# Thomasedv/RRIN

Hardware: AMD Instinct MI355X
Metric: interpolated frames/sec at 1280x720 fp32 (Net.forward, frame pairs/s) (higher is better)
Workload: dtype f32

## Files before the change

rrin_amd/csrc/conv_winoc42.hip:

```cpp
#include <type_traits>

#include "common.hpp"

#ifndef RRIN_WINO42_AGPR
#define RRIN_WINO42_AGPR 0
#endif
namespace rrin {

typedef float w42f16 __attribute__((ext_vector_type(16)));
typedef float w42f4 __attribute__((ext_vector_type(4)));

template <int PCW_>
struct W42 {
  static constexpr int PCW = PCW_;
  static constexpr int PRW = 32 / PCW;
  static constexpr int TW = 4 * PCW;
  static constexpr int TH = 2 * PRW;
  static constexpr int RC = TW + 2;
  static constexpr int WM = (RC + 3) / 4;
  static constexpr int RW = PCW == 8 ? 36 : 22;
  static_assert(RW >= 4 * WM, "raw row slots");
  static constexpr int RG = (TH + 2) * RW;
  static constexpr int RAW = 2 * RG;
  static constexpr int PIECES = (RAW + 255) / 256;
  static constexpr int STAGE = PIECES * 256;
  static constexpr int NS = 3;
  static constexpr int XP = 65;
  static constexpr int XREC = 4 * 16 * XP;
  static constexpr size_t LDS = (size_t)(NS * STAGE > XREC ? NS * STAGE : XREC) * 16;
};
static_assert(W42<8>::LDS == kWinoC42Lds && W42<4>::LDS == kWinoC42Lds, "LDS size (common.hpp)");
static_assert(2 * kWinoC42Lds <= 160 * 1024, "two blocks per CU");
struct W42P {
  static constexpr int XP = 66;
  static constexpr int XREC = 4 * 8 * XP;
  static constexpr size_t LDS = (size_t)(XREC + W42<8>::NS * W42<8>::STAGE) * 16;
};
static_assert(2 * W42P::LDS <= 160 * 1024, "two blocks per CU (persistent)");

template <int WM>
__device__ constexpr int w42_slot(int col) { return (col & 3) * WM + (col >> 2); }

__device__ inline __amdgpu_buffer_rsrc_t w42_rsrc(const void* base) {
  const uint64_t p = (uint64_t)base;
  const uint64_t u = ((uint64_t)(uint32_t)__builtin_amdgcn_readfirstlane((int)(p >> 32)) << 32) |
                     (uint32_t)__builtin_amdgcn_readfirstlane((int)(uint32_t)p);
  return __builtin_amdgcn_make_buffer_rsrc((void*)u, 0, 0x7fffffff, 0x00020000);
}

template <int EPI, int PCW, bool PERSIST>
__global__ __launch_bounds__(256, 2) void conv3x3_winoc42_kernel(ConvH8Args a) {
  using G = W42<PCW>;
  static_assert(!PERSIST || PCW == 8, "persistent tiles: the 32 x 8 geometry");
  constexpr int TH = G::TH, TW = G::TW, RG = G::RG, RW = G::RW, STAGE = G::STAGE, P = G::PIECES, WM = G::WM;
  constexpr int SB = PERSIST ? W42P::XREC : 0;
  extern __shared__ __attribute__((aligned(16))) uint4 smem4[];
  const int tid = threadIdx.x, lane = tid & 63;
  const int yw = __builtin_amdgcn_readfirstlane(tid >> 6);
  const int j = lane & 31, hh = lane >> 5;
  const int pc = j % PCW, pr = j / PCW;
  int bid;
  {
    const int nwg = (int)gridDim.x, q = nwg >> 3, r = nwg & 7;
    const int xcd = blockIdx.x & 7, slot = blockIdx.x >> 3;
    bid = (xcd < r ? xcd * (q + 1) : r * (q + 1) + (xcd - r) * q) + slot;
  }
  const int ntiles = a.co_blocks * a.tiles_x * a.tiles_y * a.n;
  if (bid >= ntiles) return;
  const int nch = a.nchunks;
  auto decode = [&](int tile, int& cob_, int& x0_, int& y0_, int& img_) {
    const int cpg = a.cob_group > 0 ? a.cob_group : a.co_blocks;
    const int gsz = cpg * (ntiles / a.co_blocks);
    const int g = tile / gsz;
    const int r = tile - g * gsz;
    const int cg = min(cpg, a.co_blocks - g * cpg);
    cob_ = g * cpg + r % cg;
    int t = r / cg;
    x0_ = (t % a.tiles_x) * TW;
    t /= a.tiles_x;
    y0_ = (t % a.tiles_y) * TH;
    img_ = t / a.tiles_y;
  };
  int tile = bid, cob, x0, y0, img;
  decode(tile, cob, x0, y0, img);

  auto tile_base = [&](int img_, int y0_, int x0_) {
    return a.src_hi + (int64_t)img_ * a.src_img + (int64_t)y0_ * a.src_wp + x0_ + (kH8PadLeft - 1);
  };
  const uint4* tbase = tile_base(img, y0, x0);
  static_assert(P <= 4, "DMA pieces");
  uint32_t voff[4];
#pragma unroll
  for (int it = 0; it < P; ++it) {
    const int idx = tid + 256 * it;
    const int g = idx >= RG ? 1 : 0;
    const int rem = idx < G::RAW ? idx - g * RG : 0;
    const int r = rem / RW, pos = rem - r * RW;
    const int m = pos / WM, q = pos - m * WM;
    const int col = 4 * q + m;
    const bool ok = idx < G::RAW && m < 4 && col < G::RC;
    voff[it] = ok ? (uint32_t)((int64_t)g * a.src_gp + (int64_t)r * a.src_wp + col) * 16u : 0u;
  }
  const int64_t chunk_stride = 2 * a.src_gp;
  auto issue_raw_at = [&](const uint4* base, int s) {
    const auto rs = w42_rsrc(base);
#pragma unroll
    for (int it = 0; it < P; ++it)
      __builtin_amdgcn_raw_ptr_buffer_load_lds(
          rs, (__attribute__((address_space(3))) void*)(smem4 + SB + s * STAGE + 256 * it + 64 * yw), 16, voff[it], 0, 0,
          0);
  };
  const uint4* raw_next = tbase;

  auto u_base = [&](int cob_) { return a.w_hi + (int64_t)cob_ * nch * 1536; };
  const uint4* ub = u_base(cob);
  const uint32_t uvoff = (uint32_t)(hh * 32 + j) * 16u;
  auto load_u = [&](int c, int x) {
    const int soff = c * (1536 * 16) + (6 * yw + (x & 4)) * 1024;
    return __builtin_bit_cast(w42f4,
                              __builtin_amdgcn_raw_buffer_load_b128(w42_rsrc(ub), uvoff + (x & 3) * 1024, soff, 0));
  };

  const int ra = yw == 0 ? 0 : (yw == 2 ? 2 : 1);
  const int rb = yw == 0 ? 2 : (yw == 1 ? 2 : (yw == 2 ? 1 : 3));
  const float sg = yw == 1 ? 1.f : -1.f;
  const int lbase = hh * RG + 2 * pr * RW + pc;
  const int oa = lbase + ra * RW, ob = lbase + rb * RW;

  w42f16 acc[6];
  w42f4 ua[6];
  w42f4 v[6];
  w42f4 d[12];

  auto read_raw = [&](int s) {
    const uint4* rw = smem4 + SB + s * STAGE;
#pragma unroll
    for (int k = 0; k < 6; ++k) {
      d[2 * k] = __builtin_bit_cast(w42f4, rw[oa + w42_slot<WM>(k)]);
      d[2 * k + 1] = __builtin_bit_cast(w42f4, rw[ob + w42_slot<WM>(k)]);
    }
  };
  w42f4 t[6];
  auto rows = [&]() {
#pragma unroll
    for (int k = 0; k < 6; ++k)
#pragma unroll
      for (int e = 0; e < 4; ++e) t[k][e] = fmaf(sg, d[2 * k + 1][e], d[2 * k][e]);
  };
  auto cols_a = [&]() {
#pragma unroll
    for (int e = 0; e < 4; ++e) {
      v[0][e] = fmaf(4.f, t[0][e], fmaf(-5.f, t[2][e], t[4][e]));
      v[1][e] = fmaf(-4.f, t[1][e] + t[2][e], t[3][e] + t[4][e]);
      v[2][e] = fmaf(4.f, t[1][e] - t[2][e], t[4][e] - t[3][e]);
    }
  };
  auto cols_b = [&]() {
#pragma unroll
    for (int e = 0; e < 4; ++e) {
      const float p = t[1][e] - t[3][e], s = t[4][e] - t[2][e];
      v[3][e] = fmaf(-2.f, p, s);
      v[4][e] = fmaf(2.f, p, s);
      v[5][e] = fmaf(4.f, t[1][e], fmaf(-5.f, t[3][e], t[5][e]));
    }
  };
  auto mfma_point = [&](const w42f4(&u)[6], int x, const bool first) {
#pragma unroll
    for (int e = 0; e < 4; ++e)
      acc[x] = __builtin_amdgcn_mfma_f32_32x32x2f32(u[x][e], v[x][e], first && e == 0 ? w42f16{} : acc[x], 0, 0, 0);
  };
  auto bar = [&]() { asm volatile("s_waitcnt lgkmcnt(0)\n\ts_barrier" ::: "memory"); };
  auto fence = [&]() { __builtin_amdgcn_sched_barrier(0); };

  auto chunk = [&](int c, int s, const bool more, const bool first, w42f4(&u)[6]) {
    const int cu = c + 1;
#pragma unroll
    for (int x = 0; x < 3; ++x) {
      mfma_point(u, x, first);
      if (more) u[x] = load_u(cu, x);
      fence();
    }
    if (more) {
      if (first)
        RRIN_VMWAIT(0, 9);
      else
        RRIN_VMWAIT(0, 6);
      bar();
      issue_raw_at(raw_next, s == 0 ? 2 : s - 1);
      if (c + 3 < nch) raw_next += chunk_stride;
      read_raw(s == 2 ? 0 : s + 1);
    }
    fence();
    mfma_point(u, 3, first);
    if (more) u[3] = load_u(cu, 3);
    fence();
    mfma_point(u, 4, first);
    if (more) u[4] = load_u(cu, 4);
    fence();
    if (more) {
      rows();
      cols_a();
    }
    fence();
    mfma_point(u, 5, first);
    if (more) u[5] = load_u(cu, 5);
    fence();
    if (more) cols_b();
  };
  auto next_stage = [](int s) { return s == 2 ? 0 : s + 1; };

  auto issue_prologue_raw = [&]() {
    issue_raw_at(tbase, 0);
    issue_raw_at(nch > 1 ? tbase + chunk_stride : tbase, 1);
    vm_fence();
  };
  auto issue_prologue_u = [&]() {
#pragma unroll
    for (int x = 0; x < 6; ++x) ua[x] = load_u(0, x);
    vm_fence();
  };
  issue_prologue_raw();
  issue_prologue_u();

  constexpr int NPR = 32 / TW;
  const int xo = lane & (TW - 1), cx = xo & 3;
  const int prw = yw * NPR + (NPR == 1 ? 0 : (lane >> 4) & 1);
  const int src = (xo >> 2) + PCW * prw + 32 * hh;
  auto qrec = [&](int k) {
    w42f4 g;
#pragma unroll
    for (int e = 0; e < 4; ++e) {
      const int vi = 4 * k + e, c = vi >> 4, i = vi & 15;
      const float m0 = acc[0][i], m1 = acc[1][i], m2 = acc[2][i], m3 = acc[3][i], m4 = acc[4][i], m5 = acc[5][i];
      g[e] = c == 0   ? (m0 + (m1 + m2)) + (m3 + m4)
             : c == 1 ? fmaf(2.f, m3 - m4, m1 - m2)
             : c == 2 ? fmaf(4.f, m3 + m4, m1 + m2)
                      : fmaf(8.f, m3 - m4, m1 - m2) + m5;
    }
    return g;
  };
  w42f4* X = reinterpret_cast<w42f4*>(smem4);
  float bsv[16];
  int ncob = 0;
  auto epilogue = [&](auto pf) {
    float yv[2][16];
    if constexpr (!PERSIST) {
      constexpr int XP = G::XP;
#pragma unroll
      for (int k = 0; k < 16; ++k) X[(yw * 16 + k) * XP + lane] = qrec(k);
      __syncthreads();
#pragma unroll
      for (int k4 = 0; k4 < 4; ++k4) {
        const int k = 4 * cx + k4;
        const w42f4 q0 = X[(0 * 16 + k) * XP + src];
        const w42f4 q1 = X[(1 * 16 + k) * XP + src];
        const w42f4 q2 = X[(2 * 16 + k) * XP + src];
        const w42f4 q3 = X[(3 * 16 + k) * XP + src];
#pragma unroll
        for (int e = 0; e < 4; ++e) {
          yv[0][4 * k4 + e] = (q0[e] + q1[e]) + q2[e];
          yv[1][4 * k4 + e] = (q1[e] - q2[e]) - q3[e];
        }
      }
    } else {
      constexpr int XP = W42P::XP;
#pragma unroll
      for (int h = 0; h < 2; ++h) {
#pragma unroll
        for (int kk = 0; kk < 8; ++kk) X[(yw * 8 + kk) * XP + lane] = qrec(4 * (kk >> 1) + 2 * h + (kk & 1));
        __syncthreads();
#pragma unroll
        for (int k4h = 0; k4h < 2; ++k4h) {
          const int kk = 2 * cx + k4h, k4 = 2 * h + k4h;
          const w42f4 q0 = X[(0 * 8 + kk) * XP + src];
          const w42f4 q1 = X[(1 * 8 + kk) * XP + src];
          const w42f4 q2 = X[(2 * 8 + kk) * XP + src];
          const w42f4 q3 = X[(3 * 8 + kk) * XP + src];
#pragma unroll
          for (int e = 0; e < 4; ++e) {
            yv[0][4 * k4 + e] = (q0[e] + q1[e]) + q2[e];
            yv[1][4 * k4 + e] = (q1[e] - q2[e]) - q3[e];
          }
        }
        if (h == 0) __syncthreads();
      }
      if constexpr (decltype(pf)::value) {
        ub = u_base(ncob);
        issue_prologue_u();
      }
    }
    uint4* dst = a.dst_hi + (int64_t)img * a.dst_img;
    auto store4 = [&](int64_t rec, const float* vv) {
      dst[rec] = make_uint4(__float_as_uint(vv[0]), __float_as_uint(vv[1]), __float_as_uint(vv[2]), __float_as_uint(vv[3]));
    };
    const int x = x0 + xo, yb = y0 + 2 * prw;
    if constexpr (EPI == RRIN_EPI_SUBPIXEL) {
      const int HH = 2 * a.h, WW = 2 * a.w, creal = a.cout >> 2;
  #pragma unroll
      for (int r = 0; r < 2; ++r) {
        const int y = yb + r;
        if (cob * 32 < a.cout && y < a.h && x < a.w) {
  #pragma unroll
          for (int qq = 0; qq < 4; ++qq) {
            const int Y = 2 * y + (qq >> 1), XX = 2 * x + (qq & 1);
            const int64_t ri = ring_index(Y, XX, HH, WW);
            if (ri >= 0) {
  #pragma unroll
              for (int e = 0; e < 4; ++e)
                a.edge[((int64_t)img * creal + cob * 8 + 4 * hh + e) * a.ring + ri] = yv[r][4 * qq + e];
            } else {
              float vv[4];
  #pragma unroll
              for (int e = 0; e < 4; ++e) vv[e] = yv[r][4 * qq + e] + bsv[4 * qq + e];
              store4((int64_t)(2 * cob + hh) * a.dst_gp + (int64_t)(Y + 1) * a.dst_wp + XX + kH8PadLeft, vv);
            }
          }
        }
      }
    } else {
      float vv[2][16];
  #pragma unroll
      for (int r = 0; r < 2; ++r) {
        const int y = yb + r;
  #pragma unroll
        for (int i = 0; i < 16; ++i) {
          float tv = yv[r][i] + bsv[i];
          if constexpr (EPI != RRIN_EPI_LINEAR) tv = leaky(tv, a.slope);
          vv[r][i] = tv;
        }
  #pragma unroll
        for (int qq = 0; qq < 4; ++qq) {
          if (cob * 32 + 8 * qq < a.cout && y < a.h && x < a.w) {
            const int64_t rec = (int64_t)(cob * 8 + 2 * qq + hh) * a.dst_gp + (int64_t)(y + 1) * a.dst_wp + x + kH8PadLeft;
            store4(rec, &vv[r][4 * qq]);
            if constexpr (EPI == RRIN_EPI_LEAKY_REP) {
              const int dy0 = y == 0 ? -1 : 0, dy1 = y == a.h - 1 ? 1 : 0;
              const int dx0 = x == 0 ? -1 : 0, dx1 = x == a.w - 1 ? 1 : 0;
              for (int dy = dy0; dy <= dy1; ++dy)
                for (int dx = dx0; dx <= dx1; ++dx)
                  if (dy | dx) store4(rec + (int64_t)dy * a.dst_wp + dx, &vv[r][4 * qq]);
            }
          }
        }
      }
      if constexpr (EPI == RRIN_EPI_LEAKY_POOL) {
        const int yp = yb;
        uint4* pdst = a.pool_hi + (int64_t)img * a.pool_img;
  #pragma unroll
        for (int qq = 0; qq < 4; ++qq) {
          float s4[4];
  #pragma unroll
          for (int e = 0; e < 4; ++e) {
            const float col = vv[0][4 * qq + e] + vv[1][4 * qq + e];
            const float nb = __int_as_float(__builtin_amdgcn_mov_dpp(__float_as_int(col), 0xB1, 0xF, 0xF, false));
            s4[e] = 0.25f * (col + nb);
          }
          if ((xo & 1) == 0 && cob * 32 + 8 * qq < a.cout && yp < a.h && x < a.w) {
            const int64_t rec =
                (int64_t)(cob * 8 + 2 * qq + hh) * a.pool_gp + (int64_t)(yp / 2 + 1) * a.pool_wp + x / 2 + kH8PadLeft;
            pdst[rec] = make_uint4(__float_as_uint(s4[0]), __float_as_uint(s4[1]), __float_as_uint(s4[2]),
                                   __float_as_uint(s4[3]));
          }
        }
      }
    }
  };

  for (;;) {
    raw_next = tbase + (nch > 2 ? 2 : nch - 1) * chunk_stride;
    RRIN_VMWAIT(P, 6);
    bar();
    read_raw(0);
    rows();
    cols_a();
    cols_b();
    {
      int s = 0;
      if (nch > 1) {
        chunk(0, s, true, true, ua);
        s = next_stage(s);
        for (int c = 1; c + 1 < nch; ++c) {
          chunk(c, s, true, false, ua);
          s = next_stage(s);
        }
        chunk(nch - 1, s, false, false, ua);
      } else {
        chunk(0, s, false, true, ua);
      }
    }
    asm volatile("s_waitcnt vmcnt(0)" ::: "memory");
#pragma unroll
    for (int i = 0; i < 16; ++i) bsv[i] = a.bias[cob * 32 + 8 * (i >> 2) + 4 * hh + (i & 3)];
    vm_fence();
#if RRIN_WINO42_AGPR
    asm volatile("" ::"a"(acc[0][0]));
#endif
    __syncthreads();
    if constexpr (!PERSIST) {
      epilogue(std::false_type{});
      break;
    } else {
      const int next = tile + (int)gridDim.x;
      const bool more = next < ntiles;
      int nx0, ny0, nimg;
      decode(more ? next : tile, ncob, nx0, ny0, nimg);
      tbase = tile_base(nimg, ny0, nx0);
      issue_prologue_raw();
      epilogue(std::true_type{});
      if (!more) break;
      tile = next;
      cob = ncob, x0 = nx0, y0 = ny0, img = nimg;
    }
  }
  if constexpr (PERSIST) asm volatile("s_waitcnt vmcnt(0)" ::: "memory");
}

template <int EPI, int PCW, bool PERSIST>
static int launch_winoc42_k(const ConvH8Args& a, int64_t grid, hipStream_t st) {
  auto k = conv3x3_winoc42_kernel<EPI, PCW, PERSIST>;
  constexpr size_t lds = PERSIST ? W42P::LDS : kWinoC42Lds;
  static LdsAttr attr;
  if (int e = attr.ensure((const void*)k, (int)lds, st)) return e;
  hipLaunchKernelGGL(k, dim3((unsigned)grid), dim3(256), lds, st, a);
  return hip_code(hipGetLastError());
}

#ifndef RRIN_WINO42_GEOM_DEFAULT
#define RRIN_WINO42_GEOM_DEFAULT 0
#endif
static std::atomic<int> g_wino42_geom{RRIN_WINO42_GEOM_DEFAULT};

#ifndef RRIN_WINO42_PERSIST_MAXCH
#define RRIN_WINO42_PERSIST_MAXCH 8
#endif
#ifndef RRIN_WINO42_PERSIST_WG
#define RRIN_WINO42_PERSIST_WG 512
#endif
#ifndef RRIN_WINO42_PERSIST_MINT
#define RRIN_WINO42_PERSIST_MINT 768
#endif

#ifndef RRIN_WINO42_UGROUP_KB
#define RRIN_WINO42_UGROUP_KB 2048
#endif
int launch_winoc42(const ConvH8Args& a, int epi, hipStream_t st) {
  ConvH8Args b = a;
  const int64_t per_cob = (int64_t)a.nchunks * 1536 * 16;
  b.cob_group = 0;
  if (RRIN_WINO42_UGROUP_KB > 0 && (int64_t)a.co_blocks * per_cob > (int64_t)RRIN_WINO42_UGROUP_KB * 1024) {
    int g = 1;
    while (2 * g < a.co_blocks && 2 * g * per_cob <= (int64_t)RRIN_WINO42_UGROUP_KB * 1024) g *= 2;
    b.cob_group = g;
  }
  const int64_t per_tile = (int64_t)a.co_blocks * a.n;
  const int64_t wide = per_tile * a.tiles_x * a.tiles_y;
  const int64_t tall = per_tile * ((a.w + 15) / 16) * ((a.h + 15) / 16);
  const int mode = g_wino42_geom.load(std::memory_order_relaxed);
  const bool use_tall = mode == 2 || (mode == 0 && (tall + 511) / 512 < (wide + 511) / 512);
  if (use_tall) {
    b.tiles_x = (a.w + 15) / 16;
    b.tiles_y = (a.h + 15) / 16;
  }
  const bool persist = !use_tall && mode != 3 && RRIN_WINO42_PERSIST_MAXCH > 0 &&
                       a.nchunks <= RRIN_WINO42_PERSIST_MAXCH && wide >= RRIN_WINO42_PERSIST_MINT;
  const int64_t grid = persist ? std::min<int64_t>(RRIN_WINO42_PERSIST_WG, wide / 2) : use_tall ? tall : wide;
#define RRIN_W42_CASE(E)                                                       \
  case E:                                                                      \
    return use_tall  ? launch_winoc42_k<E, 4, false>(b, grid, st)              \
           : persist ? launch_winoc42_k<E, 8, true>(b, grid, st)               \
                     : launch_winoc42_k<E, 8, false>(b, grid, st);
  switch (epi) {
    RRIN_W42_CASE(RRIN_EPI_LINEAR)
    RRIN_W42_CASE(RRIN_EPI_LEAKY)
    RRIN_W42_CASE(RRIN_EPI_LEAKY_POOL)
    RRIN_W42_CASE(RRIN_EPI_LEAKY_REP)
    RRIN_W42_CASE(RRIN_EPI_SUBPIXEL)
  }
#undef RRIN_W42_CASE
  return RRIN_E_ARG;
}

}

using namespace rrin;

extern "C" int rrin_conv_h8_set_wino42_geom(int32_t mode) {
  if (mode < 0 || mode > 3) return RRIN_E_ARG;
  return g_wino42_geom.exchange(mode);
}

extern "C" int64_t rrin_pack_conv3x3_wino42_floats(int32_t cout, int32_t cin) {
  if (cout < 1 || cin < 1) return RRIN_E_ARG;
  return (int64_t)((cout + 31) / 32) * ((cin + 7) / 8) * 24 * 2 * 32 * 4;
}

extern "C" int rrin_pack_conv3x3_wino42(const float* w, const float* b, int32_t cout, int32_t cin, const int32_t* perm,
                                        float* wpack, float* bpack) {
  if (!w || !b || !wpack || !bpack || cout < 1 || cin < 1) return RRIN_E_ARG;
  if (perm)
    for (int c = 0; c < cin; ++c)
      if (perm[c] < 0 || perm[c] >= cin) return RRIN_E_ARG;
  static const double G2[4][3] = {{1.0, 0.0, 0.0}, {0.5, 0.5, 0.5}, {0.5, -0.5, 0.5}, {0.0, 0.0, 1.0}};
  static const double G4[6][3] = {{0.25, 0.0, 0.0},
                                  {-1.0 / 6, -1.0 / 6, -1.0 / 6},
                                  {-1.0 / 6, 1.0 / 6, -1.0 / 6},
                                  {1.0 / 24, 1.0 / 12, 1.0 / 6},
                                  {1.0 / 24, -1.0 / 12, 1.0 / 6},
                                  {0.0, 0.0, 1.0}};
  const int cob_n = (cout + 31) / 32, nch = (cin + 7) / 8;
  int64_t o = 0;
  for (int cob = 0; cob < cob_n; ++cob)
    for (int c = 0; c < nch; ++c)
      for (int xi = 0; xi < 24; ++xi)
        for (int hh = 0; hh < 2; ++hh)
          for (int col = 0; col < 32; ++col)
            for (int e = 0; e < 4; ++e) {
              const int co = cob * 32 + col, ch = c * 8 + hh * 4 + e;
              double u = 0.0;
              if (co < cout && ch < cin) {
                const float* g = w + ((int64_t)co * cin + (perm ? perm[ch] : ch)) * 9;
                for (int ky = 0; ky < 3; ++ky)
                  for (int kx = 0; kx < 3; ++kx) u += G2[xi / 6][ky] * G4[xi % 6][kx] * (double)g[ky * 3 + kx];
              }
              wpack[o++] = (float)u;
            }
  for (int co = 0; co < cob_n * 32; ++co) bpack[co] = co < cout ? b[co] : 0.f;
  return 0;
}
```

Before: 167.1.

## Stream raw tiles continuously across persistent Winograd tiles with contiguous tile ranges

In the persistent Winograd 4x2 conv kernel, each workgroup now takes a contiguous range of tiles instead of a strided one, and tiles are decoded y-fastest so neighbouring tiles share a weight block. Input DMA becomes one continuous stream that prefetches the next tile's first chunks during the last chunk of the current tile, replacing the prologue reissue between tiles. Bias is loaded only when the output-channel block changes, and the epilogue barriers become lighter lgkmcnt+s_barrier waits. The aim is to hide the pipeline drain and refill between tiles; the stage index now carries across tiles, which adds complexity in the stage bookkeeping.

Result: slower. 160.1 (-4.1%).

```diff
diff --git a/rrin_amd/csrc/conv_winoc42.hip b/rrin_amd/csrc/conv_winoc42.hip
--- a/rrin_amd/csrc/conv_winoc42.hip
+++ b/rrin_amd/csrc/conv_winoc42.hip
@@ -74,14 +74,28 @@
     const int g = tile / gsz;
     const int r = tile - g * gsz;
     const int cg = min(cpg, a.co_blocks - g * cpg);
-    cob_ = g * cpg + r % cg;
-    int t = r / cg;
-    x0_ = (t % a.tiles_x) * TW;
-    t /= a.tiles_x;
-    y0_ = (t % a.tiles_y) * TH;
-    img_ = t / a.tiles_y;
-  };
-  int tile = bid, cob, x0, y0, img;
+    if constexpr (PERSIST) {
+      int t = r / a.tiles_y;
+      y0_ = (r - t * a.tiles_y) * TH;
+      cob_ = g * cpg + t % cg;
+      t /= cg;
+      x0_ = (t % a.tiles_x) * TW;
+      img_ = t / a.tiles_x;
+    } else {
+      cob_ = g * cpg + r % cg;
+      int t = r / cg;
+      x0_ = (t % a.tiles_x) * TW;
+      t /= a.tiles_x;
+      y0_ = (t % a.tiles_y) * TH;
+      img_ = t / a.tiles_y;
+    }
+  };
+  int tile = bid, tend = ntiles, cob, x0, y0, img;
+  if constexpr (PERSIST) {
+    const int nwg = (int)gridDim.x, q = ntiles / nwg, r = ntiles - q * nwg;
+    tile = bid * q + min(bid, r);
+    tend = tile + q + (bid < r ? 1 : 0);
+  }
   decode(tile, cob, x0, y0, img);
 
   auto tile_base = [&](int img_, int y0_, int x0_) {
@@ -111,6 +125,21 @@
           0);
   };
   const uint4* raw_next = tbase;
+  int ftile = tile, fch = 0;
+  const uint4* fbase = tbase;
+  auto issue_stream = [&](int s) {
+    issue_raw_at(fbase, s);
+    if (fch + 1 < nch) {
+      ++fch;
+      fbase += chunk_stride;
+    } else if (ftile + 1 < tend) {
+      ++ftile;
+      fch = 0;
+      int fc, fx, fy, fi;
+      decode(ftile, fc, fx, fy, fi);
+      fbase = tile_base(fi, fy, fx);
+    }
+  };
 
   auto u_base = [&](int cob_) { return a.w_hi + (int64_t)cob_ * nch * 1536; };
   const uint4* ub = u_base(cob);
@@ -131,6 +160,8 @@
   w42f4 ua[6];
   w42f4 v[6];
   w42f4 d[12];
+  float bsv[16];
+  int bcob = -1;
 
   auto read_raw = [&](int s) {
     const uint4* rw = smem4 + SB + s * STAGE;
@@ -186,9 +217,22 @@
       else
         RRIN_VMWAIT(0, 6);
       bar();
-      issue_raw_at(raw_next, s == 0 ? 2 : s - 1);
-      if (c + 3 < nch) raw_next += chunk_stride;
+      if constexpr (PERSIST) {
+        issue_stream(s == 0 ? 2 : s - 1);
+      } else {
+        issue_raw_at(raw_next, s == 0 ? 2 : s - 1);
+        if (c + 3 < nch) raw_next += chunk_stride;
+      }
       read_raw(s == 2 ? 0 : s + 1);
+    } else if constexpr (PERSIST) {
+      if (cob != bcob) {
+#pragma unroll
+        for (int i = 0; i < 16; ++i) bsv[i] = a.bias[cob * 32 + 8 * (i >> 2) + 4 * hh + (i & 3)];
+        bcob = cob;
+      }
+      vm_fence();
+      issue_stream(s == 0 ? 2 : s - 1);
+      vm_fence();
     }
     fence();
     mfma_point(u, 3, first);
@@ -210,8 +254,13 @@
   auto next_stage = [](int s) { return s == 2 ? 0 : s + 1; };
 
   auto issue_prologue_raw = [&]() {
-    issue_raw_at(tbase, 0);
-    issue_raw_at(nch > 1 ? tbase + chunk_stride : tbase, 1);
+    if constexpr (PERSIST) {
+      issue_stream(0);
+      issue_stream(1);
+    } else {
+      issue_raw_at(tbase, 0);
+      issue_raw_at(nch > 1 ? tbase + chunk_stride : tbase, 1);
+    }
     vm_fence();
   };
   auto issue_prologue_u = [&]() {
@@ -240,7 +289,6 @@
     return g;
   };
   w42f4* X = reinterpret_cast<w42f4*>(smem4);
-  float bsv[16];
   int ncob = 0;
   auto epilogue = [&](auto pf) {
     float yv[2][16];
@@ -268,7 +316,7 @@
       for (int h = 0; h < 2; ++h) {
 #pragma unroll
         for (int kk = 0; kk < 8; ++kk) X[(yw * 8 + kk) * XP + lane] = qrec(4 * (kk >> 1) + 2 * h + (kk & 1));
-        __syncthreads();
+        bar();
 #pragma unroll
         for (int k4h = 0; k4h < 2; ++k4h) {
           const int kk = 2 * cx + k4h, k4 = 2 * h + k4h;
@@ -282,7 +330,7 @@
             yv[1][4 * k4 + e] = (q1[e] - q2[e]) - q3[e];
           }
         }
-        if (h == 0) __syncthreads();
+        if (h == 0) bar();
       }
       if constexpr (decltype(pf)::value) {
         ub = u_base(ncob);
@@ -366,49 +414,52 @@
     }
   };
 
+  int s = 0;
   for (;;) {
-    raw_next = tbase + (nch > 2 ? 2 : nch - 1) * chunk_stride;
+    if constexpr (!PERSIST) raw_next = tbase + (nch > 2 ? 2 : nch - 1) * chunk_stride;
     RRIN_VMWAIT(P, 6);
     bar();
-    read_raw(0);
+    read_raw(s);
     rows();
     cols_a();
     cols_b();
-    {
-      int s = 0;
-      if (nch > 1) {
-        chunk(0, s, true, true, ua);
+    if (nch > 1) {
+      chunk(0, s, true, true, ua);
+      s = next_stage(s);
+      for (int c = 1; c + 1 < nch; ++c) {
+        chunk(c, s, true, false, ua);
         s = next_stage(s);
-        for (int c = 1; c + 1 < nch; ++c) {
-          chunk(c, s, true, false, ua);
-          s = next_stage(s);
-        }
-        chunk(nch - 1, s, false, false, ua);
-      } else {
-        chunk(0, s, false, true, ua);
-      }
-    }
-    asm volatile("s_waitcnt vmcnt(0)" ::: "memory");
-#pragma unroll
-    for (int i = 0; i < 16; ++i) bsv[i] = a.bias[cob * 32 + 8 * (i >> 2) + 4 * hh + (i & 3)];
-    vm_fence();
+      }
+      if constexpr (!PERSIST) chunk(nch - 1, s, false, false, ua);
+    } else if constexpr (PERSIST) {
+#pragma unroll
+      for (int x = 0; x < 6; ++x) acc[x] = w42f16{};
+    } else {
+      chunk(0, s, false, true, ua);
+    }
+    if constexpr (PERSIST) chunk(nch - 1, s, false, false, ua);
+    if constexpr (!PERSIST) {
+      asm volatile("s_waitcnt vmcnt(0)" ::: "memory");
+#pragma unroll
+      for (int i = 0; i < 16; ++i) bsv[i] = a.bias[cob * 32 + 8 * (i >> 2) + 4 * hh + (i & 3)];
+      vm_fence();
 #if RRIN_WINO42_AGPR
-    asm volatile("" ::"a"(acc[0][0]));
-#endif
-    __syncthreads();
-    if constexpr (!PERSIST) {
+      asm volatile("" ::"a"(acc[0][0]));
+#endif
+      __syncthreads();
       epilogue(std::false_type{});
       break;
     } else {
-      const int next = tile + (int)gridDim.x;
-      const bool more = next < ntiles;
+#if RRIN_WINO42_AGPR
+      asm volatile("" ::"a"(acc[0][0]));
+#endif
+      s = next_stage(s);
+      const bool more = tile + 1 < tend;
       int nx0, ny0, nimg;
-      decode(more ? next : tile, ncob, nx0, ny0, nimg);
-      tbase = tile_base(nimg, ny0, nx0);
-      issue_prologue_raw();
+      decode(more ? tile + 1 : tile, ncob, nx0, ny0, nimg);
       epilogue(std::true_type{});
       if (!more) break;
-      tile = next;
+      ++tile;
       cob = ncob, x0 = nx0, y0 = ny0, img = nimg;
     }
   }
```
